# glennhickey/teHmm

Measured on NVIDIA B200. Metric: hmm_trellis_cells_per_sec_fwd_bwd_viterbi, higher is better.
Workload: dtype f32

## Files before the change

tehmm_b200/csrc/api.cu:

```cuda
#include "common.cuh"
#include <algorithm>
#include <cstdarg>
#include <cstdio>
#include <cstring>
#include <string>
#include <vector>

void tehmm_launch_strict_emission(cudaStream_t, const void *, int, int64_t, int, const double *, int, int, double *, double, const double *, unsigned long long *);
void tehmm_launch_strict_forward(cudaStream_t, int64_t, int, const double *, const double *, const double *, const double *, double *);
void tehmm_launch_strict_backward(cudaStream_t, int64_t, int, const double *, const double *, const double *, double *);
void tehmm_launch_strict_viterbi(cudaStream_t, int64_t, int, const double *, const double *, const double *, const double *, int16_t *, int64_t *, double *);
void tehmm_launch_strict_lneta(cudaStream_t, int64_t, int, const double *, const double *, const double *, const double *, double, const double *, double *);
void tehmm_launch_strict_accumulate(cudaStream_t, const void *, int, int64_t, int, double *, int, int, const double *, const double *);
void tehmm_launch_strict_counts(cudaStream_t, const void *, int, int, int64_t, int64_t, int, double *, int, int, const double *);
size_t tehmm_emission_table_budget(int K);
int tehmm_launch_emission(cudaStream_t, const TehmmModelDev &, const TehmmBatchDev &, int, const double *, void *, void *, double *, double *, int *, int, cudaError_t *, int64_t, int64_t);
bool tehmm_emission_rows_ok(const TehmmModelDev &, int, const double *);
cudaError_t tehmm_launch_forward(cudaStream_t, const TehmmModelDev &, const TehmmBatchDev &, int, const void *, const double *, const double *, void *, void *, void *, double *, const int *, int, int);
cudaError_t tehmm_launch_verify(cudaStream_t, const TehmmBatchDev &, int, int, void *, const void *, double, int, int, int *, int *, double *);
cudaError_t tehmm_launch_forward_logprob(cudaStream_t, const TehmmBatchDev &, int, int, const void *, const double *, const double *, double *);
cudaError_t tehmm_launch_backward(cudaStream_t, const TehmmModelDev &, const TehmmBatchDev &, int, int, const void *, const void *, const double *, void *, uint8_t *, double *, void *, void *, void *, void *, void *, const int *, int, int);
cudaError_t tehmm_launch_trans_reduce(cudaStream_t, const TehmmModelDev &, const TehmmBatchDev &, int, const void *, const void *, const void *, double *);
cudaError_t tehmm_launch_map_reduce(cudaStream_t, const TehmmBatchDev &, const double *, double *);
cudaError_t tehmm_launch_viterbi(cudaStream_t, const TehmmModelDev &, const TehmmBatchDev &, int, const void *, const double *, void *, void *, void *, const int *, int, int, const double *, double *);
bool tehmm_viterbi_dp_scores(const TehmmModelDev &, int, const double *);
cudaError_t tehmm_launch_vit_score_reduce(cudaStream_t, const TehmmBatchDev &, const double *, double *);
cudaError_t tehmm_launch_traceback(cudaStream_t, const TehmmModelDev &, const TehmmBatchDev &, int, const void *, const double *, uint8_t *, int64_t *, uint8_t *, uint8_t *, const uint8_t *, const int *, int, int);
cudaError_t tehmm_launch_tb_verify(cudaStream_t, const TehmmBatchDev &, uint8_t *, const uint8_t *, uint8_t *, int *, int *);
cudaError_t tehmm_launch_rescore(cudaStream_t, const TehmmModelDev &, const TehmmBatchDev &, const uint8_t *, const double *, const double *, double *, double *, int64_t, int64_t);
cudaError_t tehmm_launch_emission_stats(cudaStream_t, const TehmmModelDev &, const TehmmBatchDev &, int, const void *, const double *, double *, double *, int, int);
size_t tehmm_stats_smem_bytes(int tab_rows, int N, int K, int prec);
cudaError_t tehmm_launch_widen(cudaStream_t, const uint8_t *, int64_t *, int64_t);
cudaError_t tehmm_launch_forward_tile(cudaStream_t, const TehmmModelDev &, const TehmmBatchDev &, const float *, const double *, float *, float *, float *, double *, const int *, int, int, int64_t);
cudaError_t tehmm_launch_backward_tile(cudaStream_t, const TehmmModelDev &, const TehmmBatchDev &, int, const float *, const float *, float *, uint8_t *, double *, float *, float *, const int *, int, int, int64_t, int);
int tehmm_tile_warps(void);
bool tehmm_forward_umma_ok(const TehmmModelDev &, const TehmmBatchDev &, int, int64_t);
cudaError_t tehmm_launch_forward_umma(cudaStream_t, const TehmmModelDev &, const TehmmBatchDev &, const float *, const double *, float *, float *, float *, double *, int, int64_t, int *, int);
bool tehmm_backward_umma_ok(const TehmmModelDev &, const TehmmBatchDev &, int, int, int64_t);
cudaError_t tehmm_launch_backward_umma(cudaStream_t, const TehmmModelDev &, const TehmmBatchDev &, int, const float *, const float *, float *, uint8_t *, double *, float *, float *, int, int64_t, int *);
cudaError_t tehmm_launch_xi_tile(cudaStream_t, const TehmmModelDev &, const TehmmBatchDev &, const float *, const float *, double *, float *, double *, int);
size_t tehmm_xi_tile_scratch_bytes(int sms);
cudaError_t tehmm_launch_convert(cudaStream_t, int, const void *, double *, int64_t);
cudaError_t tehmm_launch_transfer_ops(cudaStream_t, const TehmmModelDev &, const TehmmChunk *, const int64_t *, int64_t, int, int, const void *, void *, double *, int);
cudaError_t tehmm_launch_ratio_fold(cudaStream_t, const TehmmModelDev &, int64_t, int, const double *, void *, double *, int);
cudaError_t tehmm_launch_ratio_diag(cudaStream_t, const TehmmModelDev &, const TehmmBatchDev &, int, const double *, const void *, double *, double *, int);
cudaError_t tehmm_launch_chain(cudaStream_t, const TehmmModelDev &, int, int, int, const int64_t *, const int64_t *, int64_t, const void *, const double *, const void *, void *);

static thread_local std::string g_err;
static int fail(int code, const char *fmt, ...)
{
    char buf[512];
    va_list ap;
    va_start(ap, fmt);
    vsnprintf(buf, sizeof buf, fmt, ap);
    va_end(ap);
    g_err = buf;
    return code;
}
void tehmm_set_error(int code, const char *msg) { (void)code; g_err = msg ? msg : ""; }
void tehmm_hostpipe_release(tehmm_ctx *c);
#define CU(x)                                                                                 \
    do {                                                                                      \
        cudaError_t e__ = (x);                                                                \
        if (e__ != cudaSuccess)                                                               \
            return fail(TEHMM_ECUDA, "%s failed: %s (%s:%d)", #x, cudaGetErrorString(e__),    \
                        __FILE__, __LINE__);                                                  \
    } while (0)

struct DevBuf {
    void *p = nullptr;
    ~DevBuf() { if (p) cudaFree(p); }
    cudaError_t alloc(size_t n) { return cudaMalloc(&p, n ? n : 1); }
    template <typename T> T *as() { return (T *)p; }
};

#define TEHMM_TRING 32
#define TEHMM_NPENDING 64
enum { TK_EMISSION, TK_FORWARD, TK_BACKWARD, TK_VITERBI_DP, TK_TRACEBACK, TK_RESCORE, TK_STATS, TK_XI, TEHMM_NTIMED };
static const char *const tk_names[TEHMM_NTIMED] = {"us_emission", "us_forward", "us_backward", "us_viterbi_dp",
                                                    "us_traceback", "us_rescore", "us_emission_stats", "us_xi"};

struct tehmm_ctx {
    int device = 0;
    int sms = 148;
    cudaStream_t stream = nullptr;
    cudaStream_t own_stream = nullptr;
    int64_t launches = 0;
    int64_t opt_chunk_tiles = 0, opt_warmup = 0, opt_max_repair = 0;
    int64_t opt_tile = 1, opt_fine_len = 0;
    int64_t opt_timing = 0;
    int64_t opt_umma = 0;
    int64_t opt_umma64 = 1;
    int *d_fault = nullptr;
    int64_t stat_umma_passes = 0;
    int64_t opt_rescore = 0;
    int64_t opt_bwd_tmap = 0;
    int64_t opt_xi_tile = 1;
    int64_t opt_fallback_after = 2;
    int64_t stat_fallbacks = 0, stat_fallback_chunks = 0, stat_noise_accepted = 0;
    double mix_rho = -1.0;
    std::vector<double> mix_A;
    int mix_N = 0;
    cudaEvent_t ev[TEHMM_NTIMED][TEHMM_TRING][2] = {};
    int ev_n[TEHMM_NTIMED] = {};
    int64_t stat_repair_fwd = 0, stat_repair_bwd = 0, stat_repair_vit = 0;
    int64_t stat_tile_passes = 0;
    int64_t stat_bad_fwd = 0, stat_bad_bwd = 0, stat_bad_vit = 0, stat_bad_tb = 0, stat_repair_tb = 0;
    int *h_nbad = nullptr;
    int64_t opt_defer = 0;
    int *h_pending = nullptr;
    int npending = 0;
    int64_t stat_deferred_checks = 0, stat_deferred_bad = 0;
    bool has_model = false;
    TehmmModelDev m{};
    void *model_blob = nullptr;
    size_t model_blob_bytes = 0;
    std::vector<unsigned char> model_key;
    bool has_batch = false;
    TehmmBatchDev b{};
    TehmmBatchDev bf{};
    std::vector<int64_t> batch_key;
    void *batch_blob = nullptr;
    size_t batch_blob_bytes = 0;
    int *d_seq_flag = nullptr;
    int64_t seq_flag_n = 0;
    int64_t max_tiles_per_chunk = 1;
    int64_t fine_len = 0;
};

extern "C" {

int tehmm_abi_version(void) { return TEHMM_ABI_VERSION; }
const char *tehmm_last_error(void) { return g_err.c_str(); }

int tehmm_device_count(void)
{
    int n = 0;
    if (cudaGetDeviceCount(&n) != cudaSuccess) { cudaGetLastError(); return 0; }
    return n;
}

int tehmm_ctx_create(int device, tehmm_ctx **out)
{
    if (!out) return fail(TEHMM_EINVAL, "out is NULL");
    int n = tehmm_device_count();
    if (n <= 0) return fail(TEHMM_ECUDA, "no CUDA device visible: libtehmm_b200 has no CPU fallback");
    if (device < 0 || device >= n) return fail(TEHMM_EINVAL, "device %d out of range (0..%d)", device, n - 1);
    CU(cudaSetDevice(device));
    tehmm_ctx *c = new tehmm_ctx();
// ... 16 lines not shown
    if (!c) return TEHMM_OK;
    cudaSetDevice(c->device);
    cudaStreamSynchronize(c->stream);
    tehmm_hostpipe_release(c);
    if (c->model_blob) cudaFree(c->model_blob);
    if (c->batch_blob) cudaFree(c->batch_blob);
    if (c->d_seq_flag) cudaFree(c->d_seq_flag);
    if (c->h_nbad) cudaFreeHost(c->h_nbad);
    if (c->h_pending) cudaFreeHost(c->h_pending);
    if (c->d_fault) cudaFree(c->d_fault);
    for (int i = 0; i < TEHMM_NTIMED; ++i)
        for (int r = 0; r < TEHMM_TRING; ++r)
            for (int j = 0; j < 2; ++j)
                if (c->ev[i][r][j]) cudaEventDestroy(c->ev[i][r][j]);
    cudaStreamDestroy(c->own_stream);
    delete c;
    return TEHMM_OK;
}

int tehmm_ctx_sync(tehmm_ctx *c)
{
    if (!c) return fail(TEHMM_EINVAL, "ctx is NULL");
    CU(cudaSetDevice(c->device));
    CU(cudaStreamSynchronize(c->stream));
    return TEHMM_OK;
}

int tehmm_ctx_set_stream(tehmm_ctx *c, uint64_t stream)
{
    if (!c) return fail(TEHMM_EINVAL, "ctx is NULL");
    CU(cudaSetDevice(c->device));
    CU(cudaStreamSynchronize(c->stream));
    c->stream = stream == UINT64_MAX ? c->own_stream : (cudaStream_t)(uintptr_t)stream;
    return TEHMM_OK;
}

uint64_t tehmm_ctx_stream(tehmm_ctx *c) { return c ? (uint64_t)(uintptr_t)c->stream : 0; }
int64_t tehmm_ctx_launch_count(tehmm_ctx *c) { return c ? c->launches : 0; }

int tehmm_ctx_set_option(tehmm_ctx *c, const char *name, int64_t v)
{
    if (!c || !name) return fail(TEHMM_EINVAL, "NULL argument");
    if (!strcmp(name, "chunk_tiles")) c->opt_chunk_tiles = v;
    else if (!strcmp(name, "warmup")) c->opt_warmup = v;
    else if (!strcmp(name, "max_repair")) c->opt_max_repair = v;
    else if (!strcmp(name, "tile")) c->opt_tile = v;
    else if (!strcmp(name, "timing")) { c->opt_timing = v; for (int i = 0; i < TEHMM_NTIMED; ++i) c->ev_n[i] = 0; }
    else if (!strcmp(name, "fine_len")) c->opt_fine_len = v;
    else if (!strcmp(name, "umma")) c->opt_umma = v;
    else if (!strcmp(name, "umma64")) c->opt_umma64 = v;
    else if (!strcmp(name, "xi_tile")) c->opt_xi_tile = v;
    else if (!strcmp(name, "defer")) c->opt_defer = v;
    else if (!strcmp(name, "bwd_tmap")) c->opt_bwd_tmap = v;
    else if (!strcmp(name, "rescore")) c->opt_rescore = v;
    else if (!strcmp(name, "fallback_after")) c->opt_fallback_after = v;
    else return fail(TEHMM_EINVAL, "unknown option %s", name);
    return TEHMM_OK;
}

static double mix_rho_of(tehmm_ctx *c)
{
    if (c->mix_rho >= 0.0) return c->mix_rho;
    const int N = c->mix_N;
    if (N <= 0 || c->mix_A.size() != (size_t)N * N) return 0.0;
    const std::vector<double> &A = c->mix_A;
    std::vector<double> pi(N, 1.0 / N), tmp(N), B((size_t)N * N), B2((size_t)N * N);
    for (int it = 0; it < 2000; ++it) {
        double sum = 0.0;
        for (int j = 0; j < N; ++j) tmp[j] = 0.0;
        for (int i = 0; i < N; ++i) {
            const double p = pi[i];
            for (int j = 0; j < N; ++j) tmp[j] += p * A[(size_t)i * N + j];
        }
        for (int j = 0; j < N; ++j) sum += tmp[j];
        for (int j = 0; j < N; ++j) pi[j] = sum > 0.0 ? tmp[j] / sum : 1.0 / N;
    }
    for (int i = 0; i < N; ++i) for (int j = 0; j < N; ++j) B[(size_t)i * N + j] = A[(size_t)i * N + j] - pi[j];
    double lognorm = 0.0;
    for (int sq = 0; sq < 8; ++sq) {
        double f = 0.0;
        for (double v : B) f += v * v;
        f = sqrt(f);
        if (!(f > 0.0)) { lognorm = -INFINITY; break; }
        for (double &v : B) v /= f;
        lognorm = 2.0 * (lognorm + log(f));
        for (int i = 0; i < N; ++i)
            for (int j = 0; j < N; ++j) { double a = 0.0; for (int k = 0; k < N; ++k) a += B[(size_t)i * N + k] * B[(size_t)k * N + j]; B2[(size_t)i * N + j] = a; }
        B.swap(B2);
    }
    if (lognorm > -INFINITY) { double f = 0.0; for (double v : B) f += v * v; lognorm += f > 0.0 ? 0.5 * log(f) : -INFINITY; }
    const double rho = lognorm > -INFINITY ? exp(lognorm / 256.0) : 0.0;
    c->mix_rho = std::min(1.0, std::max(0.0, rho));
    return c->mix_rho;
}

int64_t tehmm_ctx_get_stat(tehmm_ctx *c, const char *name)
{
    if (!c || !name) return -1;
    if (!strcmp(name, "launches")) return c->launches;
    if (!strcmp(name, "repair_passes_forward")) return c->stat_repair_fwd;
    if (!strcmp(name, "repair_passes_backward")) return c->stat_repair_bwd;
    if (!strcmp(name, "repair_passes_viterbi")) return c->stat_repair_vit;
    if (!strcmp(name, "repaired_chunks_forward")) return c->stat_bad_fwd;
    if (!strcmp(name, "repaired_chunks_backward")) return c->stat_bad_bwd;
    if (!strcmp(name, "repaired_chunks_viterbi")) return c->stat_bad_vit;
    if (!strcmp(name, "repaired_chunks_traceback")) return c->stat_bad_tb;
// ... 841 lines not shown
            return fail(TEHMM_ECUDA, "fwd_umma_kernel: a barrier wait timed out (tensor-memory protocol fault)");
        }
        if (pass == 0) adapt_warmup(c, nb, PB.nchunks);
        if (nb == 0) break;
        if (pass >= max_pass) return fail(TEHMM_ESTATE, "forward repair did not converge (%d chunks left)", nb);
        if (c->opt_fallback_after >= 0 && pass >= c->opt_fallback_after && d_ratios == nullptr && fb_rounds < TEHMM_MAX_FALLBACK_ROUNDS) {
            if (resolve_flagged(c, st, PB, prec, 0, d_blin, sv, ev, bad, (int64_t)8 << (2 * fb_rounds))) return TEHMM_ECUDA;
            tol = tolerance_after_fallback(c, prec, false);
            fb_rounds += 1;
        }
        c->stat_repair_fwd += 1; c->stat_bad_fwd += nb;
        CU(launch(1));
        c->launches += 1;
    }
    CU(tehmm_launch_forward_logprob(st, PB, prec, c->m.NP, ev, cs, lkap, d_logprob));
    c->launches += 1;
    return TEHMM_OK;
}

int tehmm_run_backward(tehmm_ctx *c, int prec, int flags, const void *d_blin, const void *d_alpha,
                       const double *d_ratios, void *d_post, uint8_t *d_map_states,
                       double *d_map_score, double *d_start_trans, void *d_scratch)
{
    RUN_PROLOGUE();
    if (!d_blin || !d_alpha || !d_scratch) return fail(TEHMM_EINVAL, "NULL argument");
    if ((flags & TEHMM_BWD_POSTERIORS) && !d_post) return fail(TEHMM_EINVAL, "POSTERIORS needs d_post");
    if ((flags & TEHMM_BWD_MAP) && (!d_map_states || !d_map_score)) return fail(TEHMM_EINVAL, "MAP needs d_map_states and d_map_score");
    if ((flags & TEHMM_BWD_TRANS) && !d_start_trans) return fail(TEHMM_EINVAL, "TRANS needs d_start_trans");
    const Scratch s = carve(c, prec);
    char *w = (char *)d_scratch;
    void *sv = w + s.start_vec, *ev = w + s.end_vec;
    double *mp = (double *)(w + s.part_a);
    int *bad = (int *)(w + s.bad), *nbad = (int *)(w + s.nbad);
    void *xi = w + s.xi, *xd = w + s.xdiag, *g0 = w + s.gamma0;
    const int grid = scan_grid(c);
    const bool xi_tile = use_tile(c, prec, d_ratios) && (flags & TEHMM_BWD_TRANS) && (flags & TEHMM_BWD_POSTERIORS) &&
                         !(flags & TEHMM_BWD_RENORM_EPS) && c->opt_xi_tile != 0;
    if (xi_tile) flags &= ~TEHMM_BWD_TRANS;
    const bool tile = use_tile(c, prec, d_ratios) && !(flags & TEHMM_BWD_TRANS);
    const bool wide_umma = c->opt_umma64 != 0 && c->opt_tile != 0 && prec == TEHMM_F32 && c->m.NS == 2 && c->m.LD == 64 &&
                           d_ratios == nullptr && c->b.nseq == 1 && !(flags & TEHMM_BWD_TRANS);
    const TehmmBatchDev &PB = (tile || wide_umma) ? c->bf : c->b;
    bool umma_used = false;
    auto launch = [&](int mode) -> cudaError_t {
        if (wide_umma && tehmm_backward_umma_ok(c->m, PB, flags, mode, c->fine_len)) {
            cudaError_t eu = tehmm_launch_backward_umma(st, c->m, PB, flags, (const float *)d_blin, (const float *)d_alpha, (float *)d_post,
                                                        d_map_states, mp, (float *)sv, (float *)ev, c->sms, c->fine_len, c->d_fault);
            if (eu == cudaSuccess) { c->stat_umma_passes += 1; umma_used = true; return eu; }
            if (eu != cudaErrorNotSupported) return eu;
            cudaGetLastError();
        }
        if (tile) {
            c->stat_tile_passes += 1;
            return tehmm_launch_backward_tile(st, c->m, PB, flags, (const float *)d_blin, (const float *)d_alpha, (float *)d_post, d_map_states, mp, (float *)sv, (float *)ev, bad, mode, c->sms, c->fine_len, (int)c->opt_bwd_tmap);
        }
        return tehmm_launch_backward(st, c->m, PB, prec, flags, d_blin, d_alpha, d_ratios, d_post, d_map_states, mp, xi, xd, g0, sv, ev, bad, mode, grid);
    };
    tk_begin(c, TK_BACKWARD);
    CU(launch(0));
    tk_end(c, TK_BACKWARD);
    c->launches += 1;
    double tol = tolerance(prec, false);
    const int64_t max_pass = c->opt_max_repair > 0 ? c->opt_max_repair : PB.nchunks + 1;
    int fb_rounds = 0;
    for (int64_t pass = 0;; ++pass) {
        CU(tehmm_launch_verify(st, PB, prec, c->m.NP, sv, ev, tol, -1, 1, bad, nbad, nullptr));
        c->launches += 1;
        int nb = 0;
        if (umma_used && pass == 0) CU(cudaMemcpyAsync(c->h_nbad + 1, c->d_fault, sizeof(int), cudaMemcpyDeviceToHost, st));
        if (read_nbad(c, nbad, &nb, !umma_used)) return TEHMM_ECUDA;
        if (umma_used && pass == 0 && c->h_nbad[1]) {
            CU(cudaMemsetAsync(c->d_fault, 0, sizeof(int), st));
            return fail(TEHMM_ECUDA, "bwd_umma_kernel: a barrier wait timed out (tensor-memory protocol fault)");
        }
        if (pass == 0) adapt_warmup(c, nb, PB.nchunks);
        if (nb == 0) break;
        if (pass >= max_pass) return fail(TEHMM_ESTATE, "backward repair did not converge (%d chunks left)", nb);
        if (c->opt_fallback_after >= 0 && pass >= c->opt_fallback_after && d_ratios == nullptr && fb_rounds < TEHMM_MAX_FALLBACK_ROUNDS) {
            if (resolve_flagged(c, st, PB, prec, 1, d_blin, sv, ev, bad, (int64_t)8 << (2 * fb_rounds))) return TEHMM_ECUDA;
            tol = tolerance_after_fallback(c, prec, false);
            fb_rounds += 1;
        }
        c->stat_repair_bwd += 1; c->stat_bad_bwd += nb;
        CU(launch(1));
        c->launches += 1;
    }
    if (flags & TEHMM_BWD_MAP) { CU(tehmm_launch_map_reduce(st, PB, mp, d_map_score)); c->launches += 1; }
    if (flags & TEHMM_BWD_TRANS) { CU(tehmm_launch_trans_reduce(st, c->m, c->b, prec, xi, xd, g0, d_start_trans)); c->launches += 1; }
    if (xi_tile) {
        tk_begin(c, TK_XI);
        CU(tehmm_launch_xi_tile(st, c->m, c->bf, (const float *)d_alpha, (const float *)d_post, (double *)xi, (float *)g0, d_start_trans, c->sms));
        tk_end(c, TK_XI);
        c->launches += 2;
    }
    return TEHMM_OK;
}

int tehmm_fold_ratios(tehmm_ctx *c, int prec, const double *d_ratios, void *d_blin, double *d_rowmax)
{
    RUN_PROLOGUE();
    if (!d_ratios || !d_blin || !d_rowmax) return fail(TEHMM_EINVAL, "NULL argument");
    CU(tehmm_launch_ratio_fold(st, c->m, c->b.total, prec, d_ratios, d_blin, d_rowmax, c->sms));
    c->launches += 1;
    return TEHMM_OK;
}

int tehmm_ratio_diag_counts(tehmm_ctx *c, int prec, const void *d_post, const double *d_ratios,
// ... 165 lines not shown
```

tehmm_b200/csrc/tile.cu:

```cuda
#include "scan.cuh"
#include <type_traits>
#include <cuda.h>
#include <cstring>

#define TILE_WARPS 8
#ifndef TEHMM_TILE_TENSOR
#define TEHMM_TILE_TENSOR 1
#endif
#ifndef FWD_NBL
#define FWD_NBL 2
#endif
#ifndef FWD_NBS
#define FWD_NBS 1
#endif
#define BWD_STAGES 5
#define TILE_STAGE_BYTES 2048
#define TILE_NEVER 0x7fffffff

struct TransFrag {
    uint32_t hi[4][4][2];
    uint32_t lo[4][4][2];
};

__device__ __forceinline__ uint32_t tf32_rna(float x)
// ... 418 lines not shown
                            sh_now[r] = 0;
                        }
                    }
                }
                scale_of(quad_max(m0), scp[0], shp[0]);
                scale_of(quad_max(m1), scp[1], shp[1]);
                if (k >= W) {
                    esum[0] += k < ke[0] ? sh_now[0] : 0;
                    esum[1] += k < ke[1] ? sh_now[1] : 0;
                    if (alpha) {
                        sts128(sbuf + s * 128, lo2(xp[0]), lo2(xp[1]), lo2(xp[2]), lo2(xp[3]));
                        sts128(sbuf + s * 128 + 16, lo2(xp[4]), lo2(xp[5]), lo2(xp[6]), lo2(xp[7]));
                        sts128(sbuf + s * 128 + 8 * rs, hi2(xp[0]), hi2(xp[1]), hi2(xp[2]), hi2(xp[3]));
                        sts128(sbuf + s * 128 + 8 * rs + 16, hi2(xp[4]), hi2(xp[5]), hi2(xp[6]), hi2(xp[7]));
                    }
                } else if (k == W - 1 && mode == 0) {
#pragma unroll
                    for (int r = 0; r < 2; ++r)
                        if (pred[r] && k >= ks[r] && k < ke[r]) store_row_vec32(start_vec + cid[r] * 32 + 8 * q, xp, r);
                }
                if (ev) {
#pragma unroll
                    for (int r = 0; r < 2; ++r)
                        if (k + 1 == ke[r]) store_row_vec32(end_vec + cid[r] * 32 + 8 * q, xp, r);
                    kev = next_event(k + 1);
                }
            }
            if (storing) issue_store(j);
        };
        for (int j = 0; j < nblk; ++j) {
            if (kev < kb + (j + 1) * TB) block_step(j, std::true_type());
            else block_step(j, std::false_type());
        }
        nblk_done += (uint32_t)nblk;
        if (alpha) {
            if (lane < 16) bulk_wait<0>();
            __syncwarp();
        }

        for (int rr = 0; rr < 16; ++rr) {
            const int64_t c = gi * 16 + rr;
            if (c >= b.nchunks) break;
            if (mode == 1 && !bad[c]) continue;
            const TehmmChunk ch = b.chunks[c];
            double ms = 0.0;
            for (int64_t tt = ch.t0 + lane; tt < ch.t1; tt += 32) ms += rowmax[tt];
            ms = warp_sum(ms);
            const int e = __shfl_sync(TEHMM_FULL, (rr & 8) ? esum[1] : esum[0], (rr & 7) * 4);
            if (lane == 0) cscale[c] = (double)e * 0.6931471805599453094 + ms;
        }
    }
}

template <int OUT>
__global__ void __launch_bounds__(TILE_WARPS * 32, 1)
bwd_tile_kernel(TehmmModelDev m, TehmmBatchDev b, int flags, const float *__restrict__ blin,
                const float *__restrict__ alpha, float *__restrict__ post,
                uint8_t *__restrict__ map_states, double *__restrict__ map_part,
                float *__restrict__ start_vec, float *__restrict__ end_vec,
                const int *__restrict__ bad, int mode, int64_t group0)
{
    constexpr bool want_post = (OUT & TEHMM_BWD_POSTERIORS) != 0;
    constexpr bool want_map = (OUT & TEHMM_BWD_MAP) != 0;
    extern __shared__ __align__(128) unsigned char tile_smem[];
    const int lane = threadIdx.x & 31, warp = threadIdx.x >> 5;
    const int g = lane >> 2, q = lane & 3;
    const int N = m.N, W = b.warmup;
    constexpr int LD = 32;
    const uint32_t slot0 = (uint32_t)__cvta_generic_to_shared(tile_smem) +
                           (uint32_t)(warp * BWD_STAGES * 2 * TILE_STAGE_BYTES + lane * 16);
    constexpr bool renorm = (OUT & TEHMM_BWD_RENORM_EPS) != 0;
    const float eps32 = 1.1920928955078125e-07f;
    const double renorm_inv = 1.0 / (1.0 + (double)N * 1.1920928955078125e-07);
    const float renorm_invf = (float)renorm_inv;

    TransFrag A;
    load_trans<true>(m, g, q, A);
    float ones[8];
#pragma unroll
    for (int i = 0; i < 8; ++i) ones[i] = 8 * q + i < N ? 1.f : 0.f;

    const int64_t ngroups = (b.nchunks + 15) / 16;
    for (int64_t gi = group0 + (int64_t)blockIdx.x * TILE_WARPS + warp; gi < ngroups;
         gi += (int64_t)gridDim.x * TILE_WARPS) {
        int ks[2], ke[2], kbv[2];
        int64_t off[2], trow[2], cid[2];
        bool exact[2], succ[2];
        int kb = TILE_NEVER, kmax = 0;
#pragma unroll
        for (int r = 0; r < 2; ++r) {
            const int64_t c = gi * 16 + g + 8 * r;
            cid[r] = c;
            bool valid = c < b.nchunks;
            if (valid && mode == 1) valid = bad[c] != 0;
            ks[r] = TILE_NEVER; ke[r] = 0; kbv[r] = TILE_NEVER; off[r] = 0; trow[r] = 0;
            exact[r] = false; succ[r] = false;
            if (valid) {
                const TehmmChunk ch = b.chunks[c];
                const int64_t rem = ch.s1 - ch.t1;
                succ[r] = rem > 0;
                if (rem == 0) { ks[r] = W; exact[r] = true; }
                else if (mode == 1) ks[r] = W;
                else if (rem <= W) { ks[r] = W - (int)rem; exact[r] = true; }
                else ks[r] = 0;
                kbv[r] = exact[r] ? ks[r] + 1 : ks[r];
                ke[r] = W + (int)(ch.t1 - ch.t0);
                trow[r] = ch.t1 - 1 + W;
                off[r] = trow[r] * LD + 8 * q;
                kb = min(kb, ks[r]);
                kmax = max(kmax, ke[r]);
            }
        }
        kb = __reduce_min_sync(TEHMM_FULL, kb);
        kmax = __reduce_max_sync(TEHMM_FULL, kmax);
        if (kmax <= 0) continue;

        auto next_event = [&](int k) -> int {
            int e = TILE_NEVER;
#pragma unroll
            for (int r = 0; r < 2; ++r) {
                if (ks[r] >= k) e = min(e, ks[r]);
                if (ke[r] - 1 >= k) e = min(e, ke[r] - 1);
            }
            return __reduce_min_sync(TEHMM_FULL, e);
        };

        u64 up[8];
        float scp[2] = {1.f, 1.f};
        double mapsum[2] = {0.0, 0.0};
#pragma unroll
        for (int c = 0; c < 8; ++c) up[c] = 0ull;

        const float *lb[2], *la[2];
        float *pp_[2];
        uint8_t *mp_[2];
#pragma unroll
        for (int r = 0; r < 2; ++r) {
            lb[r] = blin + off[r] + LD - (int64_t)kb * LD;
            la[r] = alpha + off[r] - (int64_t)kb * LD;
            pp_[r] = want_post ? post + off[r] - (int64_t)kb * LD : nullptr;
            mp_[r] = want_map ? map_states + trow[r] - kb : nullptr;
        }
        auto issue = [&](int k, int stage) {
#pragma unroll
            for (int r = 0; r < 2; ++r) {
                const uint32_t sl = slot0 + (uint32_t)(stage * 2 * TILE_STAGE_BYTES + r * 1024);
                stage_row(sl, lb[r], k >= kbv[r] && k < ke[r]);
                stage_row(sl + TILE_STAGE_BYTES, la[r], k >= W && k < ke[r]);
                lb[r] -= LD;
                la[r] -= LD;
            }
            stage_commit();
        };

        u64 prq[8];
        bool actq[2] = {false, false}, pend = false;
        auto post_out = [&](const u64 (&pr)[8], const bool (&actr)[2], int back) {
            u64 zs = 0ull;
#pragma unroll
            for (int c = 0; c < 8; ++c) zs = fadd2(zs, pr[c]);
            const float Z0 = quad_sum(lo2(zs)), Z1 = quad_sum(hi2(zs));
            const float invZ[2] = {__frcp_rn(Z0), __frcp_rn(Z1)};
#pragma unroll
            for (int r = 0; r < 2; ++r) {
                const bool act = actr[r];
                float p[8];
#pragma unroll
                for (int c = 0; c < 8; ++c) p[c] = r ? hi2(pr[c]) : lo2(pr[c]);
                if constexpr (want_map) {
                    const float best = quad_max(fmaxf(fmax3(fmax3(p[0], p[1], p[2]), p[3], p[4]), fmax3(p[5], p[6], p[7])));
                    int idx = 99;
#pragma unroll
                    for (int i = 7; i >= 0; --i)
                        if (p[i] == best) idx = 8 * q + i;
                    idx = min(idx, __shfl_xor_sync(TEHMM_FULL, idx, 1));
                    idx = min(idx, __shfl_xor_sync(TEHMM_FULL, idx, 2));
                    const float bg = act ? best * invZ[r] : 0.f;
                    mapsum[r] += renorm ? (act ? ((double)bg + (double)eps32) * renorm_inv : 0.0) : (double)bg;
                    if (act && q == 0) mp_[r][back] = (uint8_t)(idx < N ? idx : 0);
                }
                if constexpr (want_post) {
                    float gv[8];
#pragma unroll
                    for (int i = 0; i < 8; ++i) {
                        gv[i] = p[i] * invZ[r];
                        if (renorm) gv[i] = (gv[i] + eps32) * renorm_invf * ones[i];
                    }
                    store_row8(pp_[r] + (int64_t)back * LD, act, gv);
                }
            }
        };

#pragma unroll
        for (int v = 0; v < BWD_STAGES - 1; ++v) issue(kb + v, v);
        int rs = 0, ws = BWD_STAGES - 1;
        int kev = next_event(kb);
        auto clock_step = [&](const int k, auto evtag) {
            constexpr bool EVC = decltype(evtag)::value;
            issue(k + BWD_STAGES - 1, ws);
            stage_wait<BWD_STAGES - 1>();
            float at[2][8], bt[2][8];
            const uint32_t sl = slot0 + (uint32_t)(rs * 2 * TILE_STAGE_BYTES);
            stage_read(sl, bt[0]);
            stage_read(sl + 1024, bt[1]);
            stage_read(sl + TILE_STAGE_BYTES, at[0]);
            stage_read(sl + TILE_STAGE_BYTES + 1024, at[1]);
            const bool ev = EVC;
            if constexpr (EVC) {
#pragma unroll
                for (int r = 0; r < 2; ++r) {
                    if (k == ks[r] && !exact[r]) {
                        float v[8];
                        if (mode == 1) load_vec32(start_vec + cid[r] * 32 + 8 * q, v);
                        else {
#pragma unroll
                            for (int i = 0; i < 8; ++i) v[i] = ones[i];
                        }
                        set_row(up, r, v);
                        scp[r] = 1.f;
                    }
                }
            }
            u64 wp[8];
            {
                u64 bs[2][4];
#pragma unroll
                for (int r = 0; r < 2; ++r) {
                    const u64 s2 = pk2(scp[r], scp[r]);
#pragma unroll
                    for (int p = 0; p < 4; ++p) bs[r][p] = fmul2(pk2(bt[r][2 * p], bt[r][2 * p + 1]), s2);
                }
#pragma unroll
                for (int p = 0; p < 4; ++p) {
                    wp[2 * p] = pk2(lo2(up[2 * p]) * lo2(bs[0][p]), hi2(up[2 * p]) * lo2(bs[1][p]));
                    wp[2 * p + 1] = pk2(lo2(up[2 * p + 1]) * hi2(bs[0][p]), hi2(up[2 * p + 1]) * hi2(bs[1][p]));
                }
            }
            float acc[4][4];
            tile_matmul(wp, A, acc);
            if (pend) post_out(prq, actq, 1);
            float m0 = 0.f, m1 = 0.f;
#pragma unroll
            for (int nt = 0; nt < 4; ++nt) {
                up[2 * nt] = pk2(acc[nt][0], acc[nt][2]);
                up[2 * nt + 1] = pk2(acc[nt][1], acc[nt][3]);
                m0 = fmax3(m0, acc[nt][0], acc[nt][1]);
                m1 = fmax3(m1, acc[nt][2], acc[nt][3]);
            }
            if constexpr (EVC) {
#pragma unroll
                for (int r = 0; r < 2; ++r) {
                    if (k == ks[r] && exact[r]) {
                        set_row(up, r, ones);
                        if (r == 0) m0 = 1.f; else m1 = 1.f;
                    }
                }
            }
            {
                int dummy;
                scale_of(quad_max(m0), scp[0], dummy);
                scale_of(quad_max(m1), scp[1], dummy);
            }
            if (k >= W) {
#pragma unroll
                for (int c = 0; c < 8; ++c) prq[c] = pk2(lo2(up[c]) * at[0][c], hi2(up[c]) * at[1][c]);
                actq[0] = k < ke[0];
                actq[1] = k < ke[1];
                pend = true;
            } else if (k == W - 1 && mode == 0) {
#pragma unroll
                for (int r = 0; r < 2; ++r)
                    if (succ[r] && k >= ks[r] && k < ke[r]) store_row_vec32(start_vec + cid[r] * 32 + 8 * q, up, r);
            }
            if constexpr (EVC) {
#pragma unroll
                for (int r = 0; r < 2; ++r)
                    if (k + 1 == ke[r]) store_row_vec32(end_vec + cid[r] * 32 + 8 * q, up, r);
                kev = next_event(k + 1);
            }
#pragma unroll
            for (int r = 0; r < 2; ++r) {
                if constexpr (want_post) pp_[r] -= LD;
                if constexpr (want_map) mp_[r] -= 1;
            }
            rs = rs + 1 == BWD_STAGES ? 0 : rs + 1;
            ws = ws + 1 == BWD_STAGES ? 0 : ws + 1;
        };
        for (int k = kb; k < kmax;) {
            clock_step(k, std::true_type());
            ++k;
            const int stop = min(kmax, kev);
            for (; k < stop; ++k) clock_step(k, std::false_type());
        }
        stage_wait<0>();
        if (pend) post_out(prq, actq, 1);
        if constexpr (want_map) {
#pragma unroll
            for (int r = 0; r < 2; ++r)
                if (q == 0 && ke[r] > 0) map_part[cid[r]] = mapsum[r];
        }
    }
}

#define BT_TB 2
#define BT_NB 3
#define BT_BOX (16 * BT_TB * 128)
#define BT_WARP_BYTES (BT_NB * 2 * BT_BOX + 128)

template <int OUT>
__global__ void __launch_bounds__(TILE_WARPS * 32, 1)
bwd_tile_tmap_kernel(TehmmModelDev m, TehmmBatchDev b, int flags, float *__restrict__ post,
                     uint8_t *__restrict__ map_states, double *__restrict__ map_part,
                     float *__restrict__ start_vec, float *__restrict__ end_vec,
                     const __grid_constant__ CUtensorMap tmap_b1, const __grid_constant__ CUtensorMap tmap_a,
                     int lf, int64_t ngroups)
{
    constexpr bool want_post = (OUT & TEHMM_BWD_POSTERIORS) != 0;
    constexpr bool want_map = (OUT & TEHMM_BWD_MAP) != 0;
    extern __shared__ __align__(128) unsigned char tile_smem[];
    const int lane = threadIdx.x & 31, warp = threadIdx.x >> 5;
    const int g = lane >> 2, q = lane & 3;
    const int N = m.N, W = b.warmup;
    constexpr int LD = 32;
    const uint32_t wbase = (uint32_t)__cvta_generic_to_shared(tile_smem) + (uint32_t)(warp * BT_WARP_BYTES);
    const uint32_t bars = wbase + BT_NB * 2 * BT_BOX;
    const uint32_t myoff = (uint32_t)(g * BT_TB * 128 + 32 * q);
    if (lane == 0) {
#pragma unroll
        for (int i = 0; i < BT_NB; ++i) mbar_init(bars + 8 * i, 1);
        asm volatile("fence.mbarrier_init.release.cluster;" ::: "memory");
    }
    fence_async_smem();
    __syncwarp();
    uint32_t nblk_done = 0;
    const bool renorm = (flags & TEHMM_BWD_RENORM_EPS) != 0;
    const float eps32 = 1.1920928955078125e-07f;
    const double renorm_inv = 1.0 / (1.0 + (double)N * 1.1920928955078125e-07);
    const float renorm_invf = (float)renorm_inv;

    TransFrag A;
    load_trans<true>(m, g, q, A);
    float ones[8];
#pragma unroll
    for (int i = 0; i < 8; ++i) ones[i] = 8 * q + i < N ? 1.f : 0.f;

    const int kmax = W + lf, nblk = kmax / BT_TB;
    for (int64_t gi = (int64_t)blockIdx.x * TILE_WARPS + warp; gi < ngroups;
         gi += (int64_t)gridDim.x * TILE_WARPS) {
        int64_t cid[2];
        float *pp_[2];
        uint8_t *mp_[2];
#pragma unroll
// ... 308 lines not shown
    typedef CUresult (*encode_fn)(CUtensorMap *, CUtensorMapDataType, cuuint32_t, void *, const cuuint64_t *,
                                  const cuuint64_t *, const cuuint32_t *, const cuuint32_t *, CUtensorMapInterleave,
                                  CUtensorMapSwizzle, CUtensorMapL2promotion, CUtensorMapFloatOOBfill);
    static encode_fn encode = nullptr;
    static bool tried = false;
    if (!tried) {
        tried = true;
        void *fn = nullptr;
        cudaDriverEntryPointQueryResult q;
        if (cudaGetDriverEntryPoint("cuTensorMapEncodeTiled", &fn, cudaEnableDefault, &q) == cudaSuccess &&
            q == cudaDriverEntryPointSuccess)
            encode = (encode_fn)fn;
        else
            cudaGetLastError();
    }
    if (!encode || nfull < 1 || lf < tb || lf > (1 << 30) || nfull > (1 << 30)) return false;
    const cuuint64_t dims[3] = {32, (cuuint64_t)lf, (cuuint64_t)nfull};
    const cuuint64_t strides[2] = {128, (cuuint64_t)lf * 128};
    const cuuint32_t box[3] = {32, (cuuint32_t)tb, 16}, estr[3] = {1, 1, 1};
    return encode(tm, CU_TENSOR_MAP_DATA_TYPE_FLOAT32, 3, (void *)base, dims, strides, box, estr,
                  CU_TENSOR_MAP_INTERLEAVE_NONE, CU_TENSOR_MAP_SWIZZLE_NONE, CU_TENSOR_MAP_L2_PROMOTION_L2_128B,
                  CU_TENSOR_MAP_FLOAT_OOB_FILL_NONE) == CUDA_SUCCESS;
}

cudaError_t tehmm_launch_forward_tile(cudaStream_t st, const TehmmModelDev &m, const TehmmBatchDev &b,
                                      const float *blin, const double *rowmax, float *alpha,
                                      float *start_vec, float *end_vec, double *cscale,
                                      const int *bad, int mode, int sms, int64_t fine_len)
{
    const int smem = TILE_WARPS * FWD_WARP_BYTES;
    cudaError_t e = cudaFuncSetAttribute(fwd_tile_kernel, cudaFuncAttributeMaxDynamicSharedMemorySize, smem);
    if (e != cudaSuccess) return e;
    CUtensorMap tm, tma;
    memset(&tm, 0, sizeof tm);
    memset(&tma, 0, sizeof tma);
    int lf = 0, nfull = 0;
    if (TEHMM_TILE_TENSOR && b.nseq == 1 && fine_len > 0 && mode == 0 &&
        make_lattice_tmap(&tm, blin, fine_len, b.total / fine_len) &&
        (!alpha || make_lattice_tmap(&tma, alpha, fine_len, b.total / fine_len))) {
        lf = (int)fine_len;
        nfull = (int)(b.total / fine_len);
    }
    fwd_tile_kernel<<<tile_grid(b, sms), TILE_WARPS * 32, smem, st>>>(m, b, blin, rowmax, alpha, start_vec,
                                                                      end_vec, cscale, bad, mode, tm, tma, lf, nfull);
    return cudaGetLastError();
}

static bool make_lattice_tmap_tb(CUtensorMap *tm, const float *base, int64_t lf, int64_t nfull, int tb);

cudaError_t tehmm_launch_backward_tile(cudaStream_t st, const TehmmModelDev &m, const TehmmBatchDev &b,
                                       int flags, const float *blin, const float *alpha, float *post,
                                       uint8_t *map_states, double *map_part, float *start_vec,
                                       float *end_vec, const int *bad, int mode, int sms, int64_t fine_len,
                                       int use_tmap)
{
    const int th = TILE_WARPS * 32;
    const int smem = TILE_WARPS * BWD_STAGES * 2 * TILE_STAGE_BYTES;
    const int out = flags & (TEHMM_BWD_POSTERIORS | TEHMM_BWD_MAP);
    const int outr = flags & (TEHMM_BWD_POSTERIORS | TEHMM_BWD_MAP | TEHMM_BWD_RENORM_EPS);
    int64_t group0 = 0;
    if (TEHMM_TILE_TENSOR && use_tmap && b.nseq == 1 && mode == 0 && fine_len > b.warmup && fine_len % BT_TB == 0 &&
        b.warmup % BT_TB == 0 && b.warmup >= BT_TB) {
        const int64_t lf = fine_len;
        const int64_t nfull_b = std::min<int64_t>(b.total / lf, (b.total - 1) / lf);
        const int64_t ngroups = nfull_b > 0 ? (nfull_b - 1) / 16 : 0;
        CUtensorMap tmb, tma;
        memset(&tmb, 0, sizeof tmb);
        memset(&tma, 0, sizeof tma);
        if (ngroups > 0 && make_lattice_tmap_tb(&tmb, blin + 32, lf, nfull_b, BT_TB) &&
            make_lattice_tmap_tb(&tma, alpha, lf, nfull_b, BT_TB)) {
            const int tsmem = TILE_WARPS * BT_WARP_BYTES;
            const int64_t need = (ngroups + TILE_WARPS - 1) / TILE_WARPS;
            const int tgrid = (int)(need < sms ? need : sms);
#define BWD_TMAP(O) do { cudaError_t e = cudaFuncSetAttribute(bwd_tile_tmap_kernel<O>, cudaFuncAttributeMaxDynamicSharedMemorySize, tsmem); \
                         if (e != cudaSuccess) return e; \
                         bwd_tile_tmap_kernel<O><<<tgrid, th, tsmem, st>>>(m, b, flags, post, map_states, map_part, start_vec, end_vec, tmb, tma, (int)lf, ngroups); } while (0)
            switch (out) {
            case 0: BWD_TMAP(0); break;
            case TEHMM_BWD_POSTERIORS: BWD_TMAP(TEHMM_BWD_POSTERIORS); break;
            case TEHMM_BWD_MAP: BWD_TMAP(TEHMM_BWD_MAP); break;
            default: BWD_TMAP(TEHMM_BWD_POSTERIORS | TEHMM_BWD_MAP); break;
            }
#undef BWD_TMAP
            cudaError_t e = cudaGetLastError();
            if (e != cudaSuccess) return e;
            group0 = ngroups;
        }
    }
    const int64_t left = (b.nchunks + 15) / 16 - group0;
    if (left <= 0) return cudaSuccess;
    const int64_t need = (left + TILE_WARPS - 1) / TILE_WARPS;
    const int grid = (int)(need < 1 ? 1 : (need < sms ? need : sms));
#define BWD_TILE(O) do { cudaError_t e = cudaFuncSetAttribute(bwd_tile_kernel<O>, cudaFuncAttributeMaxDynamicSharedMemorySize, smem); \
                         if (e != cudaSuccess) return e; \
                         bwd_tile_kernel<O><<<grid, th, smem, st>>>(m, b, flags, blin, alpha, post, map_states, map_part, start_vec, end_vec, bad, mode, group0); } while (0)
    switch (outr) {
    case 0: BWD_TILE(0); break;
    case TEHMM_BWD_POSTERIORS: BWD_TILE(TEHMM_BWD_POSTERIORS); break;
    case TEHMM_BWD_MAP: BWD_TILE(TEHMM_BWD_MAP); break;
    case TEHMM_BWD_POSTERIORS | TEHMM_BWD_MAP: BWD_TILE(TEHMM_BWD_POSTERIORS | TEHMM_BWD_MAP); break;
    case TEHMM_BWD_RENORM_EPS: BWD_TILE(0); break;
    case TEHMM_BWD_POSTERIORS | TEHMM_BWD_RENORM_EPS: BWD_TILE(TEHMM_BWD_POSTERIORS | TEHMM_BWD_RENORM_EPS); break;
    case TEHMM_BWD_MAP | TEHMM_BWD_RENORM_EPS: BWD_TILE(TEHMM_BWD_MAP | TEHMM_BWD_RENORM_EPS); break;
    default: BWD_TILE(TEHMM_BWD_POSTERIORS | TEHMM_BWD_MAP | TEHMM_BWD_RENORM_EPS); break;
    }
#undef BWD_TILE
    return cudaGetLastError();
}

int tehmm_tile_warps(void) { return TILE_WARPS; }

cudaError_t tehmm_launch_xi_tile(cudaStream_t st, const TehmmModelDev &m, const TehmmBatchDev &b,
                                 const float *alpha, const float *post, double *xi_part, float *gamma0,
                                 double *start_trans, int sms)
{
    const int smem = TILE_WARPS * 2 * 16 * XI_LDS * 4;
    const int64_t need = (b.nchunks + TILE_WARPS - 1) / TILE_WARPS;
    const int grid = (int)(need < 1 ? 1 : (need < sms ? need : sms));
    cudaError_t e = cudaFuncSetAttribute(xi_tile_kernel, cudaFuncAttributeMaxDynamicSharedMemorySize, smem);
    if (e != cudaSuccess) return e;
    xi_tile_kernel<<<grid, TILE_WARPS * 32, smem, st>>>(m, b, alpha, post, xi_part, gamma0);
    xi_reduce_kernel<<<(m.N * m.N + 127) / 128, 128, 0, st>>>(m, b, xi_part, grid * TILE_WARPS, gamma0, start_trans);
    return cudaGetLastError();
}
size_t tehmm_xi_tile_scratch_bytes(int sms) { return (size_t)sms * TILE_WARPS * 1024 * sizeof(double); }
```

Before: 96.17 billion.

## Add shared-memory transposed epilogue for backward tile posterior and MAP output

Adds an alternative epilogue to the backward tile kernel. It stages two clocks of alpha*beta products per warp in swizzled shared memory, then transposes them so each lane owns one row, computes the normaliser, argmax and posteriors in-lane, and writes the posteriors as coalesced float4 stores. It replaces the quad-shuffle-based post_out path and is enabled by default when posteriors are requested. The cost is extra shared memory per warp, extra syncwarps and register pressure, and a more complicated MAP tie-breaking path.

```diff
diff --git a/tehmm_b200/csrc/api.cu b/tehmm_b200/csrc/api.cu
--- a/tehmm_b200/csrc/api.cu
+++ b/tehmm_b200/csrc/api.cu
@@ -32,7 +32,7 @@
 size_t tehmm_stats_smem_bytes(int tab_rows, int N, int K, int prec);
 cudaError_t tehmm_launch_widen(cudaStream_t, const uint8_t *, int64_t *, int64_t);
 cudaError_t tehmm_launch_forward_tile(cudaStream_t, const TehmmModelDev &, const TehmmBatchDev &, const float *, const double *, float *, float *, float *, double *, const int *, int, int, int64_t);
-cudaError_t tehmm_launch_backward_tile(cudaStream_t, const TehmmModelDev &, const TehmmBatchDev &, int, const float *, const float *, float *, uint8_t *, double *, float *, float *, const int *, int, int, int64_t, int);
+cudaError_t tehmm_launch_backward_tile(cudaStream_t, const TehmmModelDev &, const TehmmBatchDev &, int, const float *, const float *, float *, uint8_t *, double *, float *, float *, const int *, int, int, int64_t, int, int);
 int tehmm_tile_warps(void);
 bool tehmm_forward_umma_ok(const TehmmModelDev &, const TehmmBatchDev &, int, int64_t);
 cudaError_t tehmm_launch_forward_umma(cudaStream_t, const TehmmModelDev &, const TehmmBatchDev &, const float *, const double *, float *, float *, float *, double *, int, int64_t, int *, int);
@@ -95,6 +95,7 @@
     int64_t stat_umma_passes = 0;
     int64_t opt_rescore = 0;
     int64_t opt_bwd_tmap = 0;
+    int64_t opt_bwd_epi = -1;
     int64_t opt_xi_tile = 1;
     int64_t opt_fallback_after = 2;
     int64_t stat_fallbacks = 0, stat_fallback_chunks = 0, stat_noise_accepted = 0;
@@ -217,6 +218,7 @@
     else if (!strcmp(name, "xi_tile")) c->opt_xi_tile = v;
     else if (!strcmp(name, "defer")) c->opt_defer = v;
     else if (!strcmp(name, "bwd_tmap")) c->opt_bwd_tmap = v;
+    else if (!strcmp(name, "bwd_epi")) c->opt_bwd_epi = v;
     else if (!strcmp(name, "rescore")) c->opt_rescore = v;
     else if (!strcmp(name, "fallback_after")) c->opt_fallback_after = v;
     else return fail(TEHMM_EINVAL, "unknown option %s", name);
@@ -1164,7 +1166,7 @@
         }
         if (tile) {
             c->stat_tile_passes += 1;
-            return tehmm_launch_backward_tile(st, c->m, PB, flags, (const float *)d_blin, (const float *)d_alpha, (float *)d_post, d_map_states, mp, (float *)sv, (float *)ev, bad, mode, c->sms, c->fine_len, (int)c->opt_bwd_tmap);
+            return tehmm_launch_backward_tile(st, c->m, PB, flags, (const float *)d_blin, (const float *)d_alpha, (float *)d_post, d_map_states, mp, (float *)sv, (float *)ev, bad, mode, c->sms, c->fine_len, (int)c->opt_bwd_tmap, (int)c->opt_bwd_epi);
         }
         return tehmm_launch_backward(st, c->m, PB, prec, flags, d_blin, d_alpha, d_ratios, d_post, d_map_states, mp, xi, xd, g0, sv, ev, bad, mode, grid);
     };
diff --git a/tehmm_b200/csrc/tile.cu b/tehmm_b200/csrc/tile.cu
--- a/tehmm_b200/csrc/tile.cu
+++ b/tehmm_b200/csrc/tile.cu
@@ -494,7 +494,16 @@
     }
 }
 
-template <int OUT>
+#define EPI_CLOCK_BYTES 2048
+#define EPI_WARP_BYTES (2 * EPI_CLOCK_BYTES + 16 * 8)
+
+__device__ __forceinline__ void lds128_32(uint32_t a, float (&v)[32], int o)
+{
+    asm volatile("ld.shared.v4.f32 {%0,%1,%2,%3}, [%4];"
+                 : "=f"(v[o]), "=f"(v[o + 1]), "=f"(v[o + 2]), "=f"(v[o + 3]) : "r"(a) : "memory");
+}
+
+template <int OUT, int EPI>
 __global__ void __launch_bounds__(TILE_WARPS * 32, 1)
 bwd_tile_kernel(TehmmModelDev m, TehmmBatchDev b, int flags, const float *__restrict__ blin,
                 const float *__restrict__ alpha, float *__restrict__ post,
@@ -504,6 +513,7 @@
 {
     constexpr bool want_post = (OUT & TEHMM_BWD_POSTERIORS) != 0;
     constexpr bool want_map = (OUT & TEHMM_BWD_MAP) != 0;
+    constexpr bool tepi = EPI == 1 && (want_post || want_map);
     extern __shared__ __align__(128) unsigned char tile_smem[];
     const int lane = threadIdx.x & 31, warp = threadIdx.x >> 5;
     const int g = lane >> 2, q = lane & 3;
@@ -511,6 +521,12 @@
     constexpr int LD = 32;
     const uint32_t slot0 = (uint32_t)__cvta_generic_to_shared(tile_smem) +
                            (uint32_t)(warp * BWD_STAGES * 2 * TILE_STAGE_BYTES + lane * 16);
+    const uint32_t ebuf = (uint32_t)__cvta_generic_to_shared(tile_smem) +
+                          (uint32_t)(TILE_WARPS * BWD_STAGES * 2 * TILE_STAGE_BYTES + warp * EPI_WARP_BYTES);
+    int64_t *const etrow = reinterpret_cast<int64_t *>(tile_smem + TILE_WARPS * BWD_STAGES * 2 * TILE_STAGE_BYTES +
+                                                       warp * EPI_WARP_BYTES + 2 * EPI_CLOCK_BYTES);
+    const int er = lane & 15, eh = lane >> 4;
+    const uint32_t ewr0 = (uint32_t)(g * 128 + (((2 * q) ^ g) << 4)), ewr1 = (uint32_t)(g * 128 + (((2 * q + 1) ^ g) << 4));
     constexpr bool renorm = (OUT & TEHMM_BWD_RENORM_EPS) != 0;
     const float eps32 = 1.1920928955078125e-07f;
     const double renorm_inv = 1.0 / (1.0 + (double)N * 1.1920928955078125e-07);
@@ -570,6 +586,17 @@
         u64 up[8];
         float scp[2] = {1.f, 1.f};
         double mapsum[2] = {0.0, 0.0};
+        int eke = 0, nq = 0, kq = 0;
+        int64_t etr = 0;
+        double emap = 0.0;
+        if constexpr (tepi) {
+            const int src = (er & 7) * 4;
+            const int ke0 = __shfl_sync(TEHMM_FULL, ke[0], src), ke1 = __shfl_sync(TEHMM_FULL, ke[1], src);
+            const int64_t t0 = __shfl_sync(TEHMM_FULL, trow[0], src), t1 = __shfl_sync(TEHMM_FULL, trow[1], src);
+            eke = er < 8 ? ke0 : ke1;
+            etr = er < 8 ? t0 : t1;
+            if (lane < 16) etrow[lane] = etr;
+        }
 #pragma unroll
         for (int c = 0; c < 8; ++c) up[c] = 0ull;
 
@@ -631,6 +658,89 @@
                     store_row8(pp_[r] + (int64_t)back * LD, act, gv);
                 }
             }
+        };
+
+        auto epi_put = [&](int k, const float (&at0)[8], const float (&at1)[8]) {
+            float p0[8], p1[8];
+#pragma unroll
+            for (int c = 0; c < 8; ++c) { p0[c] = lo2(up[c]) * at0[c]; p1[c] = hi2(up[c]) * at1[c]; }
+            const uint32_t s = ebuf + (uint32_t)(nq * EPI_CLOCK_BYTES);
+            sts128(s + ewr0, p0[0], p0[1], p0[2], p0[3]);
+            sts128(s + ewr1, p0[4], p0[5], p0[6], p0[7]);
+            sts128(s + 1024 + ewr0, p1[0], p1[1], p1[2], p1[3]);
+            sts128(s + 1024 + ewr1, p1[4], p1[5], p1[6], p1[7]);
+            if (nq == 0) kq = k;
+            ++nq;
+        };
+        auto epi_reduce = [&]() {
+            __syncwarp();
+            const int kc = kq + eh;
+            const bool act = eh < nq && kc < eke;
+            const uint32_t rb = ebuf + (uint32_t)(eh * EPI_CLOCK_BYTES + er * 128);
+            float p[32];
+#pragma unroll
+            for (int j = 0; j < 8; ++j) lds128_32(rb + (uint32_t)((j ^ (er & 7)) << 4), p, 4 * j);
+            float s[4];
+#pragma unroll
+            for (int j = 0; j < 4; ++j) {
+                s[j] = 0.f;
+#pragma unroll
+                for (int c = 0; c < 8; ++c) s[j] += p[8 * j + c];
+            }
+            const float invZ = __frcp_rn((s[0] + s[1]) + (s[2] + s[3]));
+            if constexpr (want_map) {
+                float m8[4];
+#pragma unroll
+                for (int j = 0; j < 4; ++j)
+                    m8[j] = fmaxf(fmax3(fmax3(p[8 * j], p[8 * j + 1], p[8 * j + 2]), p[8 * j + 3], p[8 * j + 4]),
+                                  fmax3(p[8 * j + 5], p[8 * j + 6], p[8 * j + 7]));
+                const float best = fmaxf(fmaxf(m8[0], m8[1]), fmaxf(m8[2], m8[3]));
+                int ij[4];
+#pragma unroll
+                for (int j = 0; j < 4; ++j) {
+                    ij[j] = 99;
+#pragma unroll
+                    for (int i = 7; i >= 0; --i)
+                        if (p[8 * j + i] == best) ij[j] = 8 * j + i;
+                }
+                const int idx = min(min(ij[0], ij[1]), min(ij[2], ij[3]));
+                if (act) map_states[etr - kc] = (uint8_t)(idx < N ? idx : 0);
+                const float bgx = act ? best * invZ : -1.f;
+                const float bgy = __shfl_down_sync(TEHMM_FULL, bgx, 16);
+                auto term = [&](float x) -> double {
+                    if (x < 0.f) return 0.0;
+                    return renorm ? ((double)x + (double)eps32) * renorm_inv : (double)x;
+                };
+                emap += term(bgx);
+                emap += term(bgy);
+            }
+            if constexpr (want_post) {
+#pragma unroll
+                for (int j = 0; j < 8; ++j) {
+                    float gv[4];
+#pragma unroll
+                    for (int i = 0; i < 4; ++i) {
+                        gv[i] = p[4 * j + i] * invZ;
+                        if (renorm) gv[i] = (gv[i] + eps32) * renorm_invf * (4 * j + i < N ? 1.f : 0.f);
+                    }
+                    sts128(rb + (uint32_t)((j ^ (er & 7)) << 4), gv[0], gv[1], gv[2], gv[3]);
+                }
+                const unsigned am = __ballot_sync(TEHMM_FULL, act);
+                __syncwarp();
+                const int sc = (lane & 8) ? 0 : 1, ch = lane & 7;
+#pragma unroll
+                for (int i = 0; i < 8; ++i) {
+                    const int R = 2 * i + eh;
+                    if ((am >> (sc * 16 + R)) & 1u) {
+                        float v[8];
+                        lds128(ebuf + (uint32_t)(sc * EPI_CLOCK_BYTES + R * 128 + ((ch ^ (R & 7)) << 4)), v, 0);
+                        const int64_t t = etrow[R] - kq - sc;
+                        *reinterpret_cast<float4 *>(post + t * LD + 4 * ch) = make_float4(v[0], v[1], v[2], v[3]);
+                    }
+                }
+            }
+            __syncwarp();
+            nq = 0;
         };
 
 #pragma unroll
@@ -680,7 +790,11 @@
             }
             float acc[4][4];
             tile_matmul(wp, A, acc);
-            if (pend) post_out(prq, actq, 1);
+            if constexpr (tepi) {
+                if (nq == 2) epi_reduce();
+            } else if (pend) {
+                post_out(prq, actq, 1);
+            }
             float m0 = 0.f, m1 = 0.f;
 #pragma unroll
             for (int nt = 0; nt < 4; ++nt) {
@@ -704,11 +818,15 @@
                 scale_of(quad_max(m1), scp[1], dummy);
             }
             if (k >= W) {
-#pragma unroll
-                for (int c = 0; c < 8; ++c) prq[c] = pk2(lo2(up[c]) * at[0][c], hi2(up[c]) * at[1][c]);
-                actq[0] = k < ke[0];
-                actq[1] = k < ke[1];
-                pend = true;
+                if constexpr (tepi) {
+                    epi_put(k, at[0], at[1]);
+                } else {
+#pragma unroll
+                    for (int c = 0; c < 8; ++c) prq[c] = pk2(lo2(up[c]) * at[0][c], hi2(up[c]) * at[1][c]);
+                    actq[0] = k < ke[0];
+                    actq[1] = k < ke[1];
+                    pend = true;
+                }
             } else if (k == W - 1 && mode == 0) {
 #pragma unroll
                 for (int r = 0; r < 2; ++r)
@@ -720,10 +838,12 @@
                     if (k + 1 == ke[r]) store_row_vec32(end_vec + cid[r] * 32 + 8 * q, up, r);
                 kev = next_event(k + 1);
             }
-#pragma unroll
-            for (int r = 0; r < 2; ++r) {
-                if constexpr (want_post) pp_[r] -= LD;
-                if constexpr (want_map) mp_[r] -= 1;
+            if constexpr (!tepi) {
+#pragma unroll
+                for (int r = 0; r < 2; ++r) {
+                    if constexpr (want_post) pp_[r] -= LD;
+                    if constexpr (want_map) mp_[r] -= 1;
+                }
             }
             rs = rs + 1 == BWD_STAGES ? 0 : rs + 1;
             ws = ws + 1 == BWD_STAGES ? 0 : ws + 1;
@@ -735,11 +855,17 @@
             for (; k < stop; ++k) clock_step(k, std::false_type());
         }
         stage_wait<0>();
-        if (pend) post_out(prq, actq, 1);
-        if constexpr (want_map) {
-#pragma unroll
-            for (int r = 0; r < 2; ++r)
-                if (q == 0 && ke[r] > 0) map_part[cid[r]] = mapsum[r];
+        if constexpr (tepi) {
+            if (nq) epi_reduce();
+            if constexpr (want_map)
+                if (lane < 16 && eke > 0) map_part[gi * 16 + er] = emap;
+        } else {
+            if (pend) post_out(prq, actq, 1);
+            if constexpr (want_map) {
+#pragma unroll
+                for (int r = 0; r < 2; ++r)
+                    if (q == 0 && ke[r] > 0) map_part[cid[r]] = mapsum[r];
+            }
         }
     }
 }
@@ -1154,7 +1280,7 @@
                                        int flags, const float *blin, const float *alpha, float *post,
                                        uint8_t *map_states, double *map_part, float *start_vec,
                                        float *end_vec, const int *bad, int mode, int sms, int64_t fine_len,
-                                       int use_tmap)
+                                       int use_tmap, int epi)
 {
     const int th = TILE_WARPS * 32;
     const int smem = TILE_WARPS * BWD_STAGES * 2 * TILE_STAGE_BYTES;
@@ -1193,20 +1319,24 @@
     if (left <= 0) return cudaSuccess;
     const int64_t need = (left + TILE_WARPS - 1) / TILE_WARPS;
     const int grid = (int)(need < 1 ? 1 : (need < sms ? need : sms));
-#define BWD_TILE(O) do { cudaError_t e = cudaFuncSetAttribute(bwd_tile_kernel<O>, cudaFuncAttributeMaxDynamicSharedMemorySize, smem); \
-                         if (e != cudaSuccess) return e; \
-                         bwd_tile_kernel<O><<<grid, th, smem, st>>>(m, b, flags, blin, alpha, post, map_states, map_part, start_vec, end_vec, bad, mode, group0); } while (0)
+    const int tsmem = smem + TILE_WARPS * EPI_WARP_BYTES;
+    if (epi < 0) epi = (flags & TEHMM_BWD_POSTERIORS) ? 1 : 0;
+#define BWD_TILE_E(O, E, S) do { cudaError_t e = cudaFuncSetAttribute(bwd_tile_kernel<O, E>, cudaFuncAttributeMaxDynamicSharedMemorySize, S); \
+                                 if (e != cudaSuccess) return e; \
+                                 bwd_tile_kernel<O, E><<<grid, th, S, st>>>(m, b, flags, blin, alpha, post, map_states, map_part, start_vec, end_vec, bad, mode, group0); } while (0)
+#define BWD_TILE(O) do { if (epi) BWD_TILE_E(O, 1, tsmem); else BWD_TILE_E(O, 0, smem); } while (0)
     switch (outr) {
-    case 0: BWD_TILE(0); break;
+    case 0: BWD_TILE_E(0, 0, smem); break;
     case TEHMM_BWD_POSTERIORS: BWD_TILE(TEHMM_BWD_POSTERIORS); break;
     case TEHMM_BWD_MAP: BWD_TILE(TEHMM_BWD_MAP); break;
     case TEHMM_BWD_POSTERIORS | TEHMM_BWD_MAP: BWD_TILE(TEHMM_BWD_POSTERIORS | TEHMM_BWD_MAP); break;
-    case TEHMM_BWD_RENORM_EPS: BWD_TILE(0); break;
+    case TEHMM_BWD_RENORM_EPS: BWD_TILE_E(0, 0, smem); break;
     case TEHMM_BWD_POSTERIORS | TEHMM_BWD_RENORM_EPS: BWD_TILE(TEHMM_BWD_POSTERIORS | TEHMM_BWD_RENORM_EPS); break;
     case TEHMM_BWD_MAP | TEHMM_BWD_RENORM_EPS: BWD_TILE(TEHMM_BWD_MAP | TEHMM_BWD_RENORM_EPS); break;
     default: BWD_TILE(TEHMM_BWD_POSTERIORS | TEHMM_BWD_MAP | TEHMM_BWD_RENORM_EPS); break;
     }
 #undef BWD_TILE
+#undef BWD_TILE_E
     return cudaGetLastError();
 }
 
```

Result: no change. 96.45 billion (median of 6 runs) (+0.3%).
